# eBay/Sequence-Semantic-Embedding

Hardware: AMD Instinct MI355X
Metric: encoded seqs/sec (+ query x target cosine-scores/sec, top-1 vs ref) (higher is better)
Workload: dtype f32; 1 GPU; configs[1]: classification stand-in, dual-encoder LSTM H=S=256 E=50 T=32 V=32000; encode 16384 source seqs/GPU/step + cosine top-10 vs 571-target index; batch_per_gpu=16384, seq_len=32, targets=571, parallelism=dp1, weights=random-init (reference initialisers, seed 0)

## Files before the change

### sequence-semantic-embedding_amd/csrc/lstm_fwd.hip

```cpp
#include <cstdlib>
#include <type_traits>

#include "sse_kernels.h"

#define LSTM_THREADS 512
#define LSTM_BM 64

#ifdef SSE_FWD_CLOCK
#include <cstdio>
__device__ long long g_fwd_clk[16 * 8];
#define FW_CLK_DECL long long ck_[8] = {0, 0, 0, 0, 0, 0, 0, 0}, ck_t = clock64();
#define FW_CLK(i)                   \
  {                                 \
    const long long n_ = clock64(); \
    ck_[i] += n_ - ck_t;            \
    ck_t = n_;                      \
  }
#else
#define FW_CLK_DECL
#define FW_CLK(i)
#endif

bool lstm_fwd_x_double(int KGx, int KGh, int RT) { return (size_t)(2 * RT * (KGx + KGh) + 1) * 1024 <= 160 * 1024; }
size_t lstm_fwd_lds_bytes(int KGx, int KGh, int RT) {
  const int xb = lstm_fwd_x_double(KGx, KGh, RT) ? 2 : 1;
  return (size_t)(xb * RT * KGx + 2 * RT * KGh) * 256 * sizeof(float) + 64 * 4 * sizeof(float);
}
static size_t lstm_fwd_xt_lds_bytes(int KGh, int RT) { return (size_t)(2 * RT * KGh) * 256 * sizeof(float) + 64 * 4 * sizeof(float); }


typedef unsigned int u32x4 __attribute__((ext_vector_type(4)));

__device__ __forceinline__ f32x4 wload(__amdgpu_buffer_rsrc_t r, int voff, int soff) {
  return __builtin_bit_cast(f32x4, __builtin_amdgcn_raw_buffer_load_b128(r, voff, soff, 0));
}

struct NoTail {
  __device__ void operator()() const {}
};
template <int MT, bool LIN, bool SWAP, int R = (MT == 1 ? 4 : 3), bool PRIO = true, typename Tail = NoTail>
__device__ __forceinline__ void gemm_pass(__amdgpu_buffer_rsrc_t wr, int voff, int soff, const float *const (&xa)[MT],
                                          const float *const (&ha)[MT], int KGx, int kend, f32x16 (&acc)[MT][2], int kbeg = 0,
                                          const Tail &tail = Tail{}) {
  auto a_frag = [&](int m, int kg) -> f32x4 {
    if constexpr (LIN) return *reinterpret_cast<const f32x4 *>(xa[m] + kg * 256);
    return *reinterpret_cast<const f32x4 *>(kg < KGx ? xa[m] + kg * 256 : ha[m] + (kg - KGx) * 256);
  };
  f32x4 p0[R], p1[R], af[R][MT];
  const int klast = kend - 1;
#pragma unroll
  for (int s = 0; s < R; ++s) {
    const int kg = kbeg + s < kend ? kbeg + s : klast;
    p0[s] = wload(wr, voff, soff + kg * 4096);
// ... 7 lines not shown
    for (int e = 0; e < 4; ++e)
#pragma unroll
      for (int m = 0; m < MT; ++m) {
        acc[m][0] = SWAP ? __builtin_amdgcn_mfma_f32_32x32x2f32(p0[s][e], af[s][m][e], acc[m][0], 0, 0, 0)
                         : __builtin_amdgcn_mfma_f32_32x32x2f32(af[s][m][e], p0[s][e], acc[m][0], 0, 0, 0);
        acc[m][1] = SWAP ? __builtin_amdgcn_mfma_f32_32x32x2f32(p1[s][e], af[s][m][e], acc[m][1], 0, 0, 0)
                         : __builtin_amdgcn_mfma_f32_32x32x2f32(af[s][m][e], p1[s][e], acc[m][1], 0, 0, 0);
      }
  };
  if constexpr (PRIO) __builtin_amdgcn_s_setprio(1);
  int kg = kbeg;
  for (; kg + R <= kend; kg += R) {
#pragma unroll
    for (int s = 0; s < R; ++s) {
      __builtin_amdgcn_sched_barrier(0);
      mfmas(s);
      __builtin_amdgcn_sched_barrier(0);
      const int kn = (kg + s + R < kend) ? kg + s + R : klast;
      p0[s] = wload(wr, voff, soff + kn * 4096);
      p1[s] = wload(wr, voff + 1024, soff + kn * 4096);
#pragma unroll
      for (int m = 0; m < MT; ++m) af[s][m] = a_frag(m, kn);
    }
  }
  if constexpr (!std::is_same_v<Tail, NoTail>) {
    __builtin_amdgcn_sched_barrier(0);
    tail();
    __builtin_amdgcn_sched_barrier(0);
  }
#pragma unroll
  for (int s = 0; s < R - 1; ++s)
    if (kg + s < kend) mfmas(s);
  if constexpr (PRIO) __builtin_amdgcn_s_setprio(0);
}

template <int RT, int MT, int UBW, bool TRAIN, bool LIN, bool SPL = false, bool TSW = false, bool XT = false>
__global__ __launch_bounds__(LSTM_THREADS) void lstm_fwd_kernel(LstmFwdArgs a) {
  static_assert(!TSW || TRAIN, "TSW is the training forward in the inference orientation");
  static_assert(!XT || (!TRAIN && LIN && !SPL), "the x table is an inference path of the linear LDS layout");
  constexpr int NTHR = LSTM_THREADS;
  extern __shared__ __attribute__((aligned(16))) float smem[];
  constexpr int ROWS = RT * 32;
  constexpr int TPR = NTHR / ROWS;
  constexpr int NWR = 8 / RT;
  constexpr bool SWAP = !TRAIN || TSW;
  const int tid = threadIdx.x, lane = tid & 63, w = tid >> 6;
  const bool split3 = !TRAIN && RT == 2 && MT == 1 && a.H > 64 && a.H <= 96;
  int ub0 = (RT == 2 && MT == 1) ? (w >> 1) : w;
  int mt0 = (RT == 2 && MT == 1) ? (w & 1) : 0;
  bool do_a = true, do_b = true;
  if (split3 && w >= 4) {
    ub0 = 2;
    mt0 = (w - 4) >> 1;
    do_a = ((w & 1) == 0);
    do_b = !do_a;
  }
  if constexpr (SPL) {
    static_assert(RT == 1 && MT == 1 && UBW == 1, "pass-split mapping is defined for one 32-row tile");
    ub0 = w & 3;
    do_a = w < 4;
    do_b = !do_a;
  }
  const int fidx = SPL ? ub0 : mt0;
  const int KGx = a.KGx, KGh = a.KGh, KG = KGx + KGh, T = a.T;
  const int KGhe = (a.KGhe > 0 && a.KGhe < KGh) ? a.KGhe : KGh;
  const int KGxs = XT ? 0 : KGx, KGs = KGxs + KGh;
  constexpr bool XD = LIN;
  auto xptr = [&](int buf, int mt) -> float * {
    return LIN ? smem + (size_t)((buf * RT + mt) * KGs) * 256 : smem + (size_t)(mt * KGx) * 256;
  };
  auto hptr = [&](int buf, int mt) -> float * {
    return LIN ? smem + (size_t)((buf * RT + mt) * KGs + KGxs) * 256
               : smem + (size_t)(RT * KGx + (buf * RT + mt) * KGh) * 256;
  };
  float *red = smem + (size_t)(LIN ? 2 * RT * KGs : RT * KGx + 2 * RT * KGh) * 256;
  const int b0 = blockIdx.x * ROWS;
  int *pass_flag = reinterpret_cast<int *>(red + 16);
  if (tid < 8) pass_flag[tid] = 0;

// ... 13 lines not shown
  for (int m = 0; m < MT; ++m) {
    const int r = b0 + (mt0 + m) * 32 + (lane & 31);
    xt_row[m] = XT && r < a.B ? (a.row_map ? a.row_map[r] : r) : -1;
  }
  auto xt_id = [&](int m, int t) -> int { return xt_row[m] >= 0 ? a.ids[(size_t)xt_row[m] * T + t] : 0; };
  auto xt_check = [&](int id) -> int {
    if (id < 0 || id >= a.V) {
      atomicOr(a.err, 1);
      id = 0;
    }
    return id;
  };
  auto x_store = [&](int buf, int kg, f32x4 lo, f32x4 hi) {
    float *dst = xptr(buf, xr >> 5) + (size_t)kg * 256;
    *reinterpret_cast<f32x4 *>(dst + (xr & 31) * 4) = lo;
    *reinterpret_cast<f32x4 *>(dst + (32 + (xr & 31)) * 4) = hi;
  };

  const int NT32 = a.NT32 > 0 ? a.NT32 : gridDim.x * RT;
  auto tape_x = [&](int ts, int kg, f32x4 lo, f32x4 hi) {
    if constexpr (TSW) {
      if (kg >= 8) return;
      sse_quad_transpose(lo, lane);
      sse_quad_transpose(hi, lane);
      const int KT = 2 + KGh / 4, b = xr & 31;
      const size_t rg = ((size_t)ts * NT32 + blockIdx.x * RT + (xr >> 5)) * 4 + (b >> 3);
      const int k0 = kg * 8 + (xr & 3);
      float *dst = a.tape_a + (rg * KT + (k0 >> 5)) * 256 + ((((b >> 2) & 1) * 32 + (k0 & 31)) << 2);
      __builtin_nontemporal_store(lo, reinterpret_cast<f32x4 *>(dst));
      __builtin_nontemporal_store(hi, reinterpret_cast<f32x4 *>(dst + 16));
    }
  };

  int t0 = 0;
  if (!TRAIN && a.pad_h != nullptr) {
    int lead = T;
    if (row_ok) {
      for (int t = xq; t < T; t += TPR)
        if (id_row[t] != 0) {
          lead = t;
          break;
        }
    }
#pragma unroll
    for (int o = 32; o > 0; o >>= 1) lead = min(lead, __shfl_xor(lead, o));
    if (lane == 0) red[w] = __int_as_float(lead);
    __syncthreads();
    lead = T;
    for (int i = 0; i < NTHR / 64; ++i) lead = min(lead, __float_as_int(red[i]));
    t0 = min(lead, T - 1);
    __syncthreads();
  }

  int xid[MT];
#pragma unroll
  for (int m = 0; m < MT; ++m) xid[m] = XT ? xt_check(xt_id(m, t0)) : 0;
  if constexpr (!XT) {
    const int id = fetch_id(t0);
    const float *src = a.emb + (size_t)id * a.Ep;
    for (int kg = xq; kg < KGx; kg += TPR) {
      f32x4 lo = *reinterpret_cast<const f32x4 *>(src + kg * 8);
      f32x4 hi = *reinterpret_cast<const f32x4 *>(src + kg * 8 + 4);
      x_store(t0 & 1, kg, lo, hi);
    }
    if constexpr (TSW) {
      for (int kg = xq; kg < 8; kg += TPR) {
        f32x4 lo = {0, 0, 0, 0}, hi = {0, 0, 0, 0};
        if (kg < KGx) {
          lo = *reinterpret_cast<const f32x4 *>(src + kg * 8);
          hi = *reinterpret_cast<const f32x4 *>(src + kg * 8 + 4);
        }
        tape_x(t0, kg, lo, hi);
      }
    }
  }
  {
    const int Hp = KGh * 8;
    for (int i = tid; i < RT * KGh * 256; i += NTHR) {
      const int mt = i / (KGh * 256), e = i % (KGh * 256);
      const int un = (e >> 8) * 8 + ((e >> 7) & 1) * 4 + (e & 3);
      hptr(t0 & 1, mt)[e] = (t0 > 0) ? a.pad_h[(size_t)t0 * Hp + un] : 0.0f;
    }
  }

  f32x16 c[UBW][MT];
#pragma unroll
  for (int u = 0; u < UBW; ++u) {
#pragma unroll
    for (int r = 0; r < 16; ++r) {
      const int un = (ub0 + 8 * u) * 32 + (SWAP ? mfma_row(r, lane) : (lane & 31));
      const float c0 = (t0 > 0) ? a.pad_c[(size_t)t0 * (KGh * 8) + un] : 0.0f;
#pragma unroll
      for (int m = 0; m < MT; ++m) c[u][m][r] = c0;
    }
  }

  if constexpr (TSW) {
    if (do_b) {
      const int KT = 2 + KGh / 4, b = lane & 31;
#pragma unroll
      for (int u = 0; u < UBW; ++u)
#pragma unroll
        for (int m = 0; m < MT; ++m) {
          const size_t rg = ((size_t)t0 * NT32 + blockIdx.x * RT + mt0 + m) * 4 + (b >> 3);
#pragma unroll
          for (int q4 = 0; q4 < 4; ++q4) {
            float *dst = a.tape_a + (rg * KT + 2 + ub0 + 8 * u) * 256 + ((((b >> 2) & 1) * 32 + q4 * 8 + (lane >> 5) * 4 + (b & 3)) << 2);
            __builtin_nontemporal_store(f32x4{0, 0, 0, 0}, reinterpret_cast<f32x4 *>(dst));
          }
        }
    }
  }
  __syncthreads();

  const __amdgpu_buffer_rsrc_t wr = __builtin_amdgcn_make_buffer_rsrc(
      const_cast<float *>(a.Wp), 0, (KGh / 4) * KG * 4096, 0x00020000);
  const int wvoff = lane * 16;
  const __amdgpu_buffer_rsrc_t xtr = __builtin_amdgcn_make_buffer_rsrc(
      const_cast<float *>(a.xtab), 0, XT ? a.V * a.xtab_ub * 512 : 0, 0x00020000);
  auto xt_load = [&](f32x16(&acc)[MT][2], const int (&id)[MT], int ub, int q) {
    const int soff = __builtin_amdgcn_readfirstlane(ub * 512 + q * 128);
#pragma unroll
    for (int m = 0; m < MT; ++m) {
      const int voff = id[m] * (a.xtab_ub * 512) + (lane >> 5) * 64;
#pragma unroll
      for (int i = 0; i < 4; ++i) {
        const f32x4 v0 = wload(xtr, voff + 16 * i, soff), v1 = wload(xtr, voff + 128 + 16 * i, soff);
#pragma unroll
        for (int e = 0; e < 4; ++e) {
          acc[m][0][4 * i + e] = v0[e];
          acc[m][1][4 * i + e] = v1[e];
        }
      }
    }
  };

  auto acc_init = [&](f32x16(&acc)[MT][2], const int (&id)[MT], int ub, int q) {
    if constexpr (XT) {
      xt_load(acc, id, ub, q);
    } else {
#pragma unroll
      for (int m = 0; m < MT; ++m)
#pragma unroll
        for (int r = 0; r < 16; ++r) {
          acc[m][0][r] = 0.0f;
          acc[m][1][r] = 0.0f;
        }
    }
  };

  constexpr bool PF = XT && RT == 2 && MT == 2 && UBW == 1;
  const bool live0 = !(a.H > 0 && ub0 * 32 >= a.H);
  f32x16 ga[MT][2], gb[MT][2];
  if (PF && live0) xt_load(ga, xid, ub0, 0);

  FW_CLK_DECL
  for (int t = t0; t < T; ++t) {
    FW_CLK(0)
    const bool have_next = (t + 1) < T;
    int nid = 0;
    f32x4 nlo = {0, 0, 0, 0}, nhi = {0, 0, 0, 0};
    int xnid[MT];
#pragma unroll
    for (int m = 0; m < MT; ++m) xnid[m] = XT && have_next ? xt_id(m, t + 1) : 0;
    if (!XT && have_next) {
      nid = fetch_id(t + 1);
      if (xq < KGx) {
        const float *src = a.emb + (size_t)nid * a.Ep + xq * 8;
        nlo = *reinterpret_cast<const f32x4 *>(src);
        nhi = *reinterpret_cast<const f32x4 *>(src + 4);
      }
    }

    const int cur = t & 1, nxt = (t + 1) & 1;
    const float *xa[MT], *ha[MT];
#pragma unroll
    for (int m = 0; m < MT; ++m) {
      xa[m] = xptr(cur, mt0 + m) + lane * 4;
      ha[m] = hptr(cur, mt0 + m) + lane * 4;
    }

    if constexpr (TRAIN && !TSW) {
      const int KT = 2 + KGh / 4;
      const int nk = 64 + KGh * 8;
      auto a_elem = [&](int mt, int kp, int b) -> float {
        if (kp >= 64) {
          const int un = kp - 64;
          return hptr(cur, mt)[(size_t)(un >> 3) * 256 + ((((un >> 2) & 1) * 32 + b) << 2) + (un & 3)];
// ... 207 lines not shown
              cn4[e] = cn;
            }
            if constexpr (TRAIN) {
              __builtin_nontemporal_store(sf4, reinterpret_cast<f32x4 *>(tp[m] + 2048 + q4 * 256));
              __builtin_nontemporal_store(so4, reinterpret_cast<f32x4 *>(tp[m] + 3072 + q4 * 256));
              __builtin_nontemporal_store(cn4, reinterpret_cast<f32x4 *>(tp[m] + 4096 + q4 * 256));
            }
          }
        }
      }
    }

    FW_CLK(6)
    if (XD) {
      __syncthreads();
      FW_CLK(7)
#pragma unroll
      for (int m = 0; m < MT; ++m)
        if (XT && !(PF && live0) && have_next) xid[m] = xt_check(xnid[m]);
    } else {
      __syncthreads();
      if (have_next) {
        if (xq < KGx) x_store(0, xq, nlo, nhi);
        for (int kg = xq + TPR; kg < KGx; kg += TPR) {
          const float *src = a.emb + (size_t)nid * a.Ep + kg * 8;
          x_store(0, kg, *reinterpret_cast<const f32x4 *>(src), *reinterpret_cast<const f32x4 *>(src + 4));
        }
        tape_x(t + 1, xq, nlo, nhi);
      }
      __syncthreads();
    }
  }

#ifdef SSE_FWD_CLOCK
  if (blockIdx.x == 0 && lane == 0)
    for (int i = 0; i < 8; ++i) g_fwd_clk[w * 8 + i] = ck_[i];
#endif
  if constexpr (TRAIN) {
    const int Hp = KGh * 8;
    for (int i = tid; i < ROWS * Hp; i += NTHR) {
      const int un = i % Hp, b = i / Hp;
      a.h_last[(size_t)(b0 + b) * Hp + un] =
          hptr(T & 1, b >> 5)[(size_t)(un >> 3) * 256 + ((((un >> 2) & 1) * 32 + (b & 31)) << 2) + (un & 3)];
    }
  }

  const int wn = w % NWR, wm = w / NWR;
  constexpr bool pwave = true;
  constexpr int PT = 16 / NWR;
  const float *hp = hptr(T & 1, wm) + lane * 4;
  f32x16 pacc[PT];
  float *ssq = hptr((T + 1) & 1, 0);
#pragma unroll
  for (int i = 0; i < PT; ++i) {
    const int nt = wn + NWR * i;
#pragma unroll
    for (int r = 0; r < 16; ++r) pacc[i][r] = 0.0f;
    if (nt < a.NTS && pwave) {
      const float *mp = a.Mp + (size_t)nt * KGh * 256 + lane * 4;
      f32x4 ax = *reinterpret_cast<const f32x4 *>(hp), bx = *reinterpret_cast<const f32x4 *>(mp), ay, by;
      int kg = 0;
      for (; kg + 1 < KGhe; kg += 2) {
        ay = *reinterpret_cast<const f32x4 *>(hp + (kg + 1) * 256);
        by = *reinterpret_cast<const f32x4 *>(mp + (kg + 1) * 256);
        __builtin_amdgcn_sched_barrier(0);
#pragma unroll
        for (int e = 0; e < 4; ++e) pacc[i] = __builtin_amdgcn_mfma_f32_32x32x2f32(ax[e], bx[e], pacc[i], 0, 0, 0);
        __builtin_amdgcn_sched_barrier(0);
        const int k2 = (kg + 2 < KGhe) ? kg + 2 : kg;
        ax = *reinterpret_cast<const f32x4 *>(hp + k2 * 256);
        bx = *reinterpret_cast<const f32x4 *>(mp + k2 * 256);
        __builtin_amdgcn_sched_barrier(0);
#pragma unroll
        for (int e = 0; e < 4; ++e) pacc[i] = __builtin_amdgcn_mfma_f32_32x32x2f32(ay[e], by[e], pacc[i], 0, 0, 0);
        __builtin_amdgcn_sched_barrier(0);
      }
      if (kg < KGhe) {
#pragma unroll
        for (int e = 0; e < 4; ++e) pacc[i] = __builtin_amdgcn_mfma_f32_32x32x2f32(ax[e], bx[e], pacc[i], 0, 0, 0);
      }
      if (a.normalize) {
#pragma unroll
        for (int r = 0; r < 16; ++r) {
          float v = pacc[i][r] * pacc[i][r];
          v += __shfl_xor(v, 1);
          v += __shfl_xor(v, 2);
          v += __shfl_xor(v, 4);
          v += __shfl_xor(v, 8);
          v += __shfl_xor(v, 16);
          if ((lane & 31) == 0) ssq[(wm * 32 + mfma_row(r, lane)) * 16 + nt] = v;
        }
      }
    }
  }
  float scale[16];
  if (a.normalize) {
    __syncthreads();
#pragma unroll
    for (int r = 0; r < 16; ++r) {
      const float *pr = ssq + (wm * 32 + mfma_row(r, lane)) * 16;
      float tot = 0.0f;
      for (int j = 0; j < a.NTS; ++j) tot += pr[j];
      scale[r] = 1.0f / sqrtf(fmaxf(tot, 1e-12f));
    }
  } else {
#pragma unroll
    for (int r = 0; r < 16; ++r) scale[r] = 1.0f;
  }
#pragma unroll
  for (int i = 0; i < PT; ++i) {
    const int nt = wn + NWR * i;
    const int col = nt * 32 + (lane & 31);
    if (nt < a.NTS && col < a.S && pwave) {
#pragma unroll
      for (int r = 0; r < 16; ++r) {
        const int row = b0 + wm * 32 + mfma_row(r, lane);
        if (row < a.B) a.out[(size_t)(a.row_map ? a.row_map[row] : row) * a.S + col] = pacc[i][r] * scale[r];
      }
    }
  }
}

template <int RT, int MT, int UBW, bool TRAIN, bool LIN, bool SPL, bool TSW = false, bool XT = false>
static hipError_t launch_one(const LstmFwdArgs &a, size_t lds, hipStream_t stream) {
  hipError_t e = hipFuncSetAttribute(reinterpret_cast<const void *>(lstm_fwd_kernel<RT, MT, UBW, TRAIN, LIN, SPL, TSW, XT>),
                                     hipFuncAttributeMaxDynamicSharedMemorySize, (int)lds);
  if (e != hipSuccess) return e;
  const dim3 grid(a.NT32 > 0 ? a.NT32 / RT : (a.B + RT * 32 - 1) / (RT * 32)), block(LSTM_THREADS);
  hipLaunchKernelGGL((lstm_fwd_kernel<RT, MT, UBW, TRAIN, LIN, SPL, TSW, XT>), grid, block, lds, stream, a);
#ifdef SSE_FWD_CLOCK
  {
    static int n = 0;
    if (a.B >= 1024 && n++ % 16 == 4) {
      long long v[128];
      (void)hipStreamSynchronize(stream);
      (void)hipMemcpyFromSymbol(v, HIP_SYMBOL(g_fwd_clk), sizeof v);
      for (int w = 0; w < 8; ++w)
        fprintf(stderr, "[fwd clock <%d,%d,%d> B=%d H=%d] wave %d cycles/step: prefetch %lld | setup %lld | passA gemm %lld | epiA+x %lld | passB gemm %lld | flag wait %lld | epiB %lld | barrier %lld\n",
                RT, MT, UBW, a.B, a.H, w, v[w * 8 + 0] / a.T, v[w * 8 + 1] / a.T, v[w * 8 + 2] / a.T, v[w * 8 + 3] / a.T, v[w * 8 + 4] / a.T, v[w * 8 + 5] / a.T,
                v[w * 8 + 6] / a.T, v[w * 8 + 7] / a.T);
    }
  }
#endif
  return hipGetLastError();
}

template <int RT, int MT, int UBW, bool SPL = false>
static hipError_t launch_cfg(const LstmFwdArgs &a_in, hipStream_t stream) {
  LstmFwdArgs a = a_in;
  a.xdouble = lstm_fwd_x_double(a.KGx, a.KGh, RT) ? 1 : 0;
  const size_t lds = lstm_fwd_lds_bytes(a.KGx, a.KGh, RT);
  const bool train = a.tape_g != nullptr;
  if constexpr (!SPL && !(RT == 2 && MT == 1)) {
    if (!train && a.xtab != nullptr) {
      if (a.xtab_ub != (a.H > 0 ? (a.H + 31) / 32 : a.KGh / 4)) return hipErrorInvalidValue;
      if ((int64_t)a.V * a.xtab_ub * 512 > INT32_MAX) return hipErrorInvalidValue;
      return launch_one<RT, MT, UBW, false, true, false, false, true>(a, lstm_fwd_xt_lds_bytes(a.KGh, RT), stream);
    }
  }
  if (train && a.tape_swap) {
    if (a.tape_a_split) return hipErrorInvalidValue;
    return a.xdouble ? launch_one<RT, MT, UBW, true, true, SPL, true>(a, lds, stream)
                     : launch_one<RT, MT, UBW, true, false, SPL, true>(a, lds, stream);
  }
  if (a.xdouble)
    return train ? launch_one<RT, MT, UBW, true, true, SPL>(a, lds, stream) : launch_one<RT, MT, UBW, false, true, SPL>(a, lds, stream);
  return train ? launch_one<RT, MT, UBW, true, false, SPL>(a, lds, stream) : launch_one<RT, MT, UBW, false, false, SPL>(a, lds, stream);
}

int lstm_fwd_rows_per_wg(int Hp, int B, int tiles_elsewhere, int cus) {
  if (cus <= 0) cus = 256;
  if (Hp == 512) return 32;
  if ((Hp == 256 || Hp == 128) && (B + 31) / 32 + tiles_elsewhere <= cus) return 32;
// ... 40 lines not shown
```

### sequence-semantic-embedding_amd/csrc/sse_api.hip

```cpp
#include <cmath>
#include <cstdarg>
#include <cstdio>
#include <cstdlib>
#include <algorithm>
#include <chrono>
#include <cstring>
#include <dlfcn.h>
#include <link.h>
#include <mutex>
#include <string>
#include <vector>

#include "../../include/sse_hip.h"
#include "sse_kernels.h"
#include "train.h"

namespace {

thread_local std::string g_create_error;

struct Variable {
  std::string name;
  int rows = 0, cols = 0;
  int64_t count = 0;
// ... 65 lines not shown
  DevBuf ids_raw[2], perm, hot_part[2];
  int perm_B = 0;
  std::vector<int32_t> h_perm, h_rows[2], h_tgt;
  std::vector<float> h_labels;
};

}

enum { PATH_PERSIST, PATH_CLUSTER, PATH_SMALL, PATH_X3, PATH_GENERIC, PATH_FWD, PATH_FWD_ROWS32, PATH_FWD_ROWS64, PATH_FWD_GS, PATH_FWD_XT,
       PATH_COUNT };
static const char *const LSTM_PATH_NAMES[PATH_COUNT] = {"lstm_path_persist", "lstm_path_cluster", "lstm_path_small", "lstm_path_x3",
                                                "lstm_path_generic", "lstm_path_fwd", "lstm_fwd_rows32", "lstm_fwd_rows64",
                                                "lstm_fwd_gate_split", "lstm_fwd_x_table"};

struct sse_handle {
  sse_config cfg;
  std::mutex mu;
  std::string err;
  std::vector<Variable> vars;
  Encoder enc[2];
  bool packed_dirty = true;
  uint64_t weights_version = 1;
  bool mp_fresh = false;
  bool pad_skip = true;
  int pad_sort_dev = 1;
  int64_t score_two_pass_min_rows = 49152, score_two_pass_rows = 524288;
  int64_t two_pass_calls = 0;
  DevBuf s_lmax;
  bool lstm_gate_split = true;
  DevBuf s_padzero, s_padwork, s_padorder;
  int32_t *pad_stat = nullptr;
  int32_t pad_seq = 0;
  int64_t pad_sorted_calls = 0;
  int64_t lstm_path_calls[10] = {0, 0, 0, 0, 0, 0, 0, 0, 0, 0};
  bool lstm_x3 = false;
  unsigned short *emb16 = nullptr;
  bool emb16_valid = false;
  int lstm_persist_rows = 32;
  uint32_t persist_epoch = 0;
  hipStream_t stream = nullptr;
  bool persist_inject = false;
  int64_t persist_fallbacks = 0;
  int cu_count = 0;
  int lstm_cluster_rows = 1024;
  uint32_t cluster_epoch = 0;
  int lstm_cluster_chunks = 3;
  int cluster_backoff = -1;
  int cluster_skip[2] = {0, 0};
  int lstm_cluster_coop = 1;
  int lstm_cluster_wt = 0;
  int lstm_cluster_drop = 0;
  int lstm_small_rows = 1024;
  int lstm_x_table = 1;
  int lstm_x_table_mb = 256;
  int64_t x_table_builds = 0;
  bool score_small_index = true;
  bool score_small_x3 = true;
  bool score_bf16 = true;
  void *idxp16 = nullptr;
  size_t idxp16_cap = 0;
  bool idxp16_valid = false;
  bool fb_cnt_init = false;
  int uncert_word = 0;
  bool cnn_bf16 = false;
  unsigned short *emb_bf16 = nullptr, *cnn_Wc16 = nullptr, *cnn_Mx3 = nullptr;
  int lstm_train_rows = 0;
// ... 391 lines not shown

static int encode_generic_locked(sse_handle *h, Encoder &e, const int32_t *ids, int B, int T, int normalize, float *out, hipStream_t st) {
  const sse_config &c = h->cfg;
  const int E = c.embedding_size, S = c.encoding_size;
  const GenLstmDims d0 = gen_lstm_dims(32, T, E, e.H);
  const size_t per_row = (size_t)T * d0.Kp * sizeof(float);
  int rows = (int)std::min<size_t>(8192, std::max<size_t>(32, (((size_t)1 << 30) / per_row) / 32 * 32));
  const GenLstmDims dm = gen_lstm_dims(std::min(rows, B), T, E, e.H);
  if (reserve(h, h->g_A, gen_lstm_a_floats(dm) * sizeof(float)) || reserve(h, h->g_G, (size_t)dm.Bp * 4 * dm.Hq * sizeof(float)) ||
      reserve(h, h->g_c, (size_t)dm.Bp * dm.Hq * sizeof(float)) || reserve(h, h->g_hl, (size_t)dm.Bp * dm.Hq * sizeof(float)) ||
      reserve(h, h->g_raw, (size_t)dm.Bp * S * sizeof(float)))
    return 1;
  const int side = (&e == &h->enc[1]) ? 1 : 0;
  if (h->g_ver[side] != h->weights_version || !h->g_KT[side].p) {
    if (reserve(h, h->g_KT[side], gen_lstm_kt_floats(dm) * sizeof(float)) || reserve(h, h->g_Kq[side], gen_lstm_kt_floats(dm) * sizeof(float)) ||
        reserve(h, h->g_MT[side], (size_t)S * dm.Hq * sizeof(float)))
      return 1;
    HIPCHECK(h, launch_gen_pack(h->vars[e.kernel].dev, h->vars[e.proj].dev, dm, S, (float *)h->g_KT[side].p, (float *)h->g_Kq[side].p,
                                (float *)h->g_MT[side].p, st));
    h->g_ver[side] = h->weights_version;
  }
  for (int b0 = 0; b0 < B; b0 += rows) {
    const int nb = std::min(rows, B - b0);
    const GenLstmDims d = gen_lstm_dims(nb, T, E, e.H);
    HIPCHECK(h, launch_gen_forward(ids + (size_t)b0 * T, h->vars[0].dev, c.vocab_size, (const float *)h->g_KT[side].p, h->vars[e.bias].dev, d,
                                   (float *)h->g_A.p, (float *)h->g_G.p, (float *)h->g_c.p, nullptr, (float *)h->g_hl.p, h->err_flag, st));
    HIPCHECK(h, launch_gen_project((const float *)h->g_hl.p, (const float *)h->g_MT[side].p, d, S, (float *)h->g_raw.p, st));
    if (normalize) HIPCHECK(h, launch_l2_normalize((const float *)h->g_raw.p, out + (size_t)b0 * S, nb, S, st));
    else HIPCHECK(h, hipMemcpyAsync(out + (size_t)b0 * S, h->g_raw.p, (size_t)nb * S * sizeof(float), hipMemcpyDeviceToDevice, st));
  }
  return 0;
}

static int device_pad_sort(sse_handle *h, int side, const int32_t *ids, int B, int T, hipStream_t st, const int32_t **row_map,
                           bool *padded) {
  if (*row_map || !h->pad_skip || h->pad_sort_dev == 0 || T < 2 || T > SSE_PAD_SORT_MAX_T || B <= 64) return 0;
  volatile int32_t *stat = h->pad_stat + 2 * side;
  const int seen = h->pad_sort_dev == 2 ? 2 : (stat[0] != 0 ? (int)stat[1] : 1);
  const bool scatter = seen != 0;
  if (!h->s_padzero.p) {
    if (reserve(h, h->s_padzero, pad_sort_zeroed_words() * sizeof(int32_t))) return 1;
    HIPCHECK(h, hipMemsetAsync(h->s_padzero.p, 0, h->s_padzero.cap, st));
  }
  if (reserve(h, h->s_padwork, pad_sort_work_words(B, T) * sizeof(int32_t))) return 1;
  if (scatter && reserve(h, h->s_padorder, (size_t)B * sizeof(int32_t))) return 1;
  h->pad_seq = h->pad_seq == INT32_MAX ? 1 : h->pad_seq + 1;
  HIPCHECK(h, launch_pad_sort(ids, B, T, (int32_t *)h->s_padzero.p, (int32_t *)h->s_padwork.p, (int32_t *)h->s_padorder.p,
                              h->pad_stat + 2 * side, h->pad_seq, scatter, st));
  if (scatter) {
    *row_map = (const int32_t *)h->s_padorder.p;
    *padded = seen == 2;
    h->pad_sorted_calls += 1;
  }
  return 0;
}

int next_epoch(sse_handle *h, DevBuf &xchg, uint32_t &epoch, size_t need, hipStream_t st, uint32_t *next) {
  if (epoch == 0 || epoch >= (1u << 20) - 1 || need > xchg.cap) {
    if (reserve(h, xchg, need)) return 1;
    HIPCHECK(h, hipMemsetAsync(xchg.p, 0, xchg.cap, st));
    epoch = 0;
  }
  *next = ++epoch;
  return 0;
}

int inject_miss(sse_handle *h, hipStream_t st) {
  static const int32_t four = 4;
  if (h->persist_inject) HIPCHECK(h, hipMemcpyAsync(h->err_flag, &four, sizeof four, hipMemcpyHostToDevice, st));
  return 0;
}

int encode_persist(sse_handle *h, int side, const int32_t *ids, int B, int T, int normalize, float *out, hipStream_t st) {
  Encoder &e = h->enc[side], &own = lstm_owner(h, e);
  if (ensure_waug(h, own, st)) return 1;
  LstmPersistArgs pa;
  fill_small_args(h, e, pa);
  pa.ids = ids;
  pa.out = out;
// ... 139 lines not shown
  if (h->lstm_x_table == 0 || own.Hp < 256) return 0;
  const int64_t V = h->cfg.vocab_size;
  const int UBt = (own.H + 31) / 32;
  const size_t bytes = lstm_xtable_floats(V, UBt) * sizeof(float);
  if (bytes > ((size_t)h->lstm_x_table_mb << 20) || bytes > (size_t)INT32_MAX) return 0;
  if (own.xtab_valid) {
    *use = true;
    return 0;
  }
  if (h->lstm_x_table == 1 && (int64_t)B * T < V) return 0;
  if (!own.xtab && hipMalloc((void **)&own.xtab, bytes) != hipSuccess) {
    (void)hipGetLastError();
    own.xtab = nullptr;
    return 0;
  }
  HIPCHECK(h, launch_lstm_xtable(h->emb_pad, own.Wp, V, own.Ep, own.KGx, own.KGh, UBt, own.xtab, st));
  own.xtab_valid = true;
  h->x_table_builds += 1;
  *use = true;
  return 0;
}

int encode_fwd(sse_handle *h, int side, const int32_t *ids, int B, int T, int normalize, float *out, const EncodeRequest &rq,
               hipStream_t st) {
  Encoder &e = h->enc[side], &own = lstm_owner(h, e);
  LstmFwdArgs a;
  fill_fwd_args(h, e, a);
  a.ids = ids;
  a.out = out;
  a.B = B;
  a.T = T;
  a.normalize = normalize ? 1 : 0;
  a.row_map = rq.row_map;
  bool padded_hint = rq.padded_hint;
  if (device_pad_sort(h, side, ids, B, T, st, &a.row_map, &padded_hint)) return 1;
  if (h->pad_skip && T > 1) {
    if (ensure_pad_table(h, own.pad_fwd, own.Hp, T, st, [&](const int32_t *zero_ids, float *scratch, int Tt) {
          LstmFwdArgs ta;
          fill_fwd_args(h, own, ta);
          ta.ids = zero_ids;
          ta.out = scratch;
          ta.B = 1;
          ta.T = Tt;
          ta.normalize = 0;
          ta.rec_h = own.pad_fwd.h;
          ta.rec_c = own.pad_fwd.c;
          HIPCHECK(h, launch_lstm_fwd(ta, own.Hp, st));
          return 0;
        }))
      return 1;
    a.pad_h = own.pad_fwd.h;
    a.pad_c = own.pad_fwd.c;
    if (padded_hint && a.row_map && e.Hp <= 256) a.force_rows = 32;
  }
  bool use_xt = false;
  if (ensure_x_table(h, own, B, T, st, &use_xt)) return 1;
  if (use_xt) {
    a.xtab = own.xtab;
    a.xtab_ub = (own.H + 31) / 32;
  }
  const int variant = lstm_fwd_variant(a, e.Hp);
  h->lstm_path_calls[(variant & 64) ? PATH_FWD_ROWS64 : PATH_FWD_ROWS32] += 1;
  if (variant & LSTM_FWD_GATE_SPLIT) h->lstm_path_calls[PATH_FWD_GS] += 1;
  if (variant & LSTM_FWD_X_TABLE) h->lstm_path_calls[PATH_FWD_XT] += 1;
  HIPCHECK(h, launch_lstm_fwd(a, e.Hp, st));
  return 0;
}

int encode_dev_locked(sse_handle *h, int side, const int32_t *ids, int B, int T, int normalize, float *out, hipStream_t st,
                      const EncodeRequest &rq = EncodeRequest()) {
  const sse_config &c = h->cfg;
  if (side != SSE_SIDE_SOURCE && side != SSE_SIDE_TARGET) return fail(h, "side must be 0 (source) or 1 (target)");
  if (B < 0 || T < 1) return fail(h, "bad batch shape B=%d T=%d", B, T);
  if (B == 0) return 0;
  if (side == SSE_SIDE_TARGET && h->tgt_table >= 0) {
    const Variable &tv = h->vars[h->tgt_table];
    if (B != tv.rows)
      return fail(h, "network mode has no target sequence encoder: tgt_seq_embedding is a [%d,%d] variable "
                     "(sse_model.py:214,233); request exactly %d rows", tv.rows, tv.cols, tv.rows);
    if (normalize) HIPCHECK(h, launch_l2_normalize(tv.dev, out, tv.rows, tv.cols, st));
    else HIPCHECK(h, hipMemcpyAsync(out, tv.dev, tv.count * sizeof(float), hipMemcpyDeviceToDevice, st));
    return 0;
  }
  if (c.network_mode == SSE_MODE_SOURCE_ONLY_CNN) {
    if (ensure_packed(h, st)) return 1;
    const int Ep = emb_cols(c);
    if (T < 5) return fail(h, "source_only_cnn needs max_seq_length >= 5 (widest filter)");
    if (cnn_lds_bytes(T, Ep, 0) > 160 * 1024)
      return fail(h, "source_only_cnn: T*E = %d*%d does not fit the LDS tile of the gfx950 kernel", T, c.embedding_size);
    if (reserve(h, h->s_feat, (size_t)((B + 31) / 32) * 72 * 256 * sizeof(float))) return 1;
    if (h->cnn_bf16) {
      const int Ep8 = round_up(c.embedding_size, 8);
      if (cnn_bf16_lds_bytes(T, Ep8, 0) > 160 * 1024)
        return fail(h, "source_only_cnn (bf16): T*E = %d*%d does not fit the LDS tile of the gfx950 kernel", T, c.embedding_size);
      HIPCHECK(h, launch_cnn_fwd_bf16(ids, h->emb_bf16, h->cnn_Wc16, h->cnn_bias, (float *)h->s_feat.p, h->err_flag, B, T,
                                      c.vocab_size, Ep8, nullptr, nullptr, st));
      HIPCHECK(h, launch_cnn_proj_x3((const float *)h->s_feat.p, h->cnn_Mx3, out, B, c.encoding_size, normalize ? 1 : 0, st));
// ... 1083 lines not shown
  if (B == 0) return 0;
  if (B < 0 || T < 1 || !ids_host || !out_scores || !out_ids) return fail(h, "bad arguments to sse_encode_score_topk");
  if (!h->idxp) return fail(h, "no index uploaded");
  if (h->cfg.encoding_size != h->idx_S)
    return fail(h, "index dimension %d != encoding_size %d", h->idx_S, h->cfg.encoding_size);
  if (encode_host_ids_locked(h, side, ids_host, B, T, normalize, true)) return 1;
  int32_t bits = 0;
  if (score_to_host_locked(h, (const float *)h->s_out.p, B, k, out_scores, out_ids, &bits)) return 1;
  if (bits) {
    if (check_err_flag(h, nullptr, &bits)) return 1;
    if (bits == 4) {
      if (encode_fallback_locked(h, side, B, T, normalize, nullptr)) return 1;
      if (score_to_host_locked(h, (const float *)h->s_out.p, B, k, out_scores, out_ids)) return 1;
    }
  }
  if (enc_out_host)
    HIPCHECK(h, hipMemcpy(enc_out_host, h->s_out.p, (size_t)B * h->cfg.encoding_size * sizeof(float), hipMemcpyDeviceToHost));
  return 0;
}

int sse_get_counter(sse_handle *h, const char *name, int64_t *value) {
  if (!h || !name || !value) return 1;
  std::lock_guard<std::mutex> lk(h->mu);
  if (strcmp(name, "lstm_persist_fallbacks") == 0) {
    *value = h->persist_fallbacks;
    return 0;
  }
  if (strcmp(name, "score_two_pass_calls") == 0) {
    *value = h->two_pass_calls;
    return 0;
  }
  if (strcmp(name, "pad_sorted_calls") == 0) {
    *value = h->pad_sorted_calls;
    return 0;
  }
  if (strcmp(name, "eval_paired_calls") == 0) {
    *value = h->eval_paired_calls;
    return 0;
  }
  if (strcmp(name, "lstm_x_table_builds") == 0) {
    *value = h->x_table_builds;
    return 0;
  }
  for (int i = 0; i < PATH_COUNT; ++i) {
    if (strcmp(name, LSTM_PATH_NAMES[i]) != 0) continue;
    *value = h->lstm_path_calls[i];
    return 0;
  }
  if (strcmp(name, "lstm_coop_refused") == 0) {
    *value = (int64_t)lstm_coop_refused();
    return 0;
  }
  static const char *const rank_names[2] = {"score_rank_band_rows", "score_rank_bruteforce_pairs"};
  for (int i = 0; i < 2; ++i) {
    if (strcmp(name, rank_names[i]) != 0) continue;
    unsigned long long v[2] = {0, 0};
    if (h->s_rk_cnt.p && h->rk_cnt_init) {
      HIPCHECK(h, hipSetDevice(h->cfg.device));
      HIPCHECK(h, hipDeviceSynchronize());
      HIPCHECK(h, hipMemcpy(v, h->s_rk_cnt.p, sizeof v, hipMemcpyDeviceToHost));
    }
    *value = (int64_t)v[i];
    return 0;
  }
  static const char *const above_names[3] = {"score_above_band_rows", "score_above_bruteforce_pairs", "score_above_long_segments"};
  for (int i = 0; i < 3; ++i) {
// ... 1485 lines not shown
```

### sequence-semantic-embedding_amd/csrc/sse_kernels.h

```cpp
#pragma once
#include <hip/hip_runtime.h>
#include <stdint.h>

typedef float f32x4 __attribute__((ext_vector_type(4)));
typedef float f32x16 __attribute__((ext_vector_type(16)));

__host__ __device__ static inline int frag32_off(int r_in_tile, int k_in_group) {
  return ((((k_in_group >> 2) << 5) + r_in_tile) << 2) + (k_in_group & 3);
}

__device__ static inline int mfma_row(int reg, int lane) { return (reg & 3) + 8 * (reg >> 2) + 4 * (lane >> 5); }

static inline int round_up(int x, int m) { return (x + m - 1) / m * m; }

typedef unsigned int sse_u32x4 __attribute__((ext_vector_type(4)));
__host__ __device__ static inline unsigned short sse_bf16_rne(float f) {
  unsigned u;
  __builtin_memcpy(&u, &f, 4);
  u += 0x7FFFu + ((u >> 16) & 1u);
  return (unsigned short)(u >> 16);
}
__host__ __device__ static inline float sse_bf16_f32(unsigned short h) {
  const unsigned u = (unsigned)h << 16;
  float f;
// ... 47 lines not shown
  (void)v;
  (void)lane;
#endif
}

#define SSE_TANH_SMALL 0.25f
__device__ __forceinline__ float sse_sigmoid(float x) { return __builtin_amdgcn_rcpf(1.0f + __builtin_amdgcn_exp2f(-1.44269504089f * x)); }
__device__ __forceinline__ float sse_tanh(float x) {
  const float big = 1.0f - 2.0f * __builtin_amdgcn_rcpf(1.0f + __builtin_amdgcn_exp2f(2.88539008178f * x));
  const float x2 = x * x;
  const float p = __builtin_fmaf(x2, __builtin_fmaf(x2, __builtin_fmaf(x2, -17.0f / 315.0f, 2.0f / 15.0f), -1.0f / 3.0f), 1.0f);
  return __builtin_fabsf(x) < SSE_TANH_SMALL ? x * p : big;
}

struct LstmFwdArgs {
  const int32_t *ids;
  const float *emb;
  const float *Wp;
  const float *Mp;
  float *out;
  int32_t *err;
  int32_t B, T, V, Ep, KGx, KGh, S, NTS, normalize;
  int32_t H = 0;
  int32_t KGhe = 0;
  int32_t NT32 = 0;
  int32_t xdouble = 1;
  int32_t tiles_elsewhere = 0;
  int32_t force_rows = 0;
  int32_t cu_count = 0;
  int32_t gate_split = 1;
  const float *pad_h = nullptr, *pad_c = nullptr;
  const int32_t *row_map = nullptr;
  float *rec_h = nullptr, *rec_c = nullptr;
  const float *xtab = nullptr;
  int32_t xtab_ub = 0;
  float *tape_g = nullptr;
  float *tape_a = nullptr;
  int32_t tape_a_split = 0;
  int32_t tape_swap = 0;
  float *h_last = nullptr;
};
size_t lstm_fwd_lds_bytes(int KGx, int KGh, int RT);
bool lstm_fwd_x_double(int KGx, int KGh, int RT);
int lstm_fwd_rows_per_wg(int Hp, int B, int tiles_elsewhere = 0, int cus = 0 );
hipError_t launch_lstm_fwd(const LstmFwdArgs &a, int Hp, hipStream_t stream);
enum { LSTM_FWD_GATE_SPLIT = 1, LSTM_FWD_X_TABLE = 2 };
int lstm_fwd_variant(const LstmFwdArgs &a, int Hp);
size_t lstm_xtable_floats(int64_t V, int UBt);
hipError_t launch_lstm_xtable(const float *emb , const float *Wp, int64_t V, int Ep, int KGx, int KGh, int UBt,
                              float *table, hipStream_t stream);
size_t lstm_fwd_gs_lds_bytes(int KGx, int NB);
bool lstm_fwd_gs_ok(int KGx, int KGh, int H);
hipError_t launch_lstm_fwd_gs(const LstmFwdArgs &a, hipStream_t stream);

struct LstmSmallArgs {
  const int32_t *ids;
  const float *emb;
  const float *Waug;
  const float *M;
  float *out;
  int32_t *err;
  int32_t B, T, V, E, H, S, normalize;
  const float *pad_h = nullptr, *pad_c = nullptr;
  float *rec_h = nullptr, *rec_c = nullptr;
  int32_t pad_stride = 0;
};
size_t lstm_small_lds_bytes(int E, int H, int S);
size_t lstm_small_waug_floats(int E, int H);
hipError_t launch_pack_lstm_small(const float *K, const float *b, int E, int H, float *out, hipStream_t stream);
hipError_t launch_lstm_small(const LstmSmallArgs &a, hipStream_t stream);

struct LstmX3Args {
  const int32_t *ids;
  const unsigned short *emb16;
  const unsigned short *Wx3;
  const float *Mp;
  float *out;
  int32_t *err;
  int32_t B, T, V, KGX, H, S, NTS, normalize;
  const int32_t *row_map = nullptr;
// ... 324 lines not shown
```

Baseline: 7.573 million seqs/s.

## Fold pad detection into LSTM forward and pipeline the output projection

When the pad-sort pass would only detect padding without scattering, detection now happens inside the LSTM forward kernel, which writes the pad status flag itself. This removes a separate detection kernel launch. The prologue also hoists the id loads and the x-table setup ahead of the pad scan, unrolls that scan four ids at a time, and zeroes the h state with vector stores when no prefix is skipped. The final projection moves to a multi-stage buffer-load pipeline with DPP row reductions. The trade-offs are added kernel complexity, a system fence on the flag write, and extra clock instrumentation behind a debug macro.

```diff
diff --git a/sequence-semantic-embedding_amd/csrc/lstm_fwd.hip b/sequence-semantic-embedding_amd/csrc/lstm_fwd.hip
--- a/sequence-semantic-embedding_amd/csrc/lstm_fwd.hip
+++ b/sequence-semantic-embedding_amd/csrc/lstm_fwd.hip
@@ -16,9 +16,21 @@
     ck_[i] += n_ - ck_t;            \
     ck_t = n_;                      \
   }
+__device__ long long g_fwd_fix[16 * 8];
+#define FX_CLK_DECL long long fx_[8] = {0, 0, 0, 0, 0, 0, 0, 0}, fx_t = clock64();
+#define FX_CLK(i)                   \
+  {                                 \
+    const long long n_ = clock64(); \
+    fx_[i] += n_ - fx_t;            \
+    fx_t = n_;                      \
+  }
+#define FX_DRAIN asm volatile("s_waitcnt vmcnt(0)" ::: "memory");
 #else
 #define FW_CLK_DECL
 #define FW_CLK(i)
+#define FX_CLK_DECL
+#define FX_CLK(i)
+#define FX_DRAIN
 #endif
 
 bool lstm_fwd_x_double(int KGx, int KGh, int RT) { return (size_t)(2 * RT * (KGx + KGh) + 1) * 1024 <= 160 * 1024; }
@@ -92,6 +104,54 @@
   for (int s = 0; s < R - 1; ++s)
     if (kg + s < kend) mfmas(s);
   if constexpr (PRIO) __builtin_amdgcn_s_setprio(0);
+}
+
+__device__ __forceinline__ float row_sum16_lane0(float v) {
+  auto dpp = [](float x, auto ctrl) {
+    return __builtin_bit_cast(float, __builtin_amdgcn_update_dpp(0, __builtin_bit_cast(int, x), decltype(ctrl)::value, 0xf, 0xf, true));
+  };
+  v += dpp(v, std::integral_constant<int, 0xB1>{});
+  v += dpp(v, std::integral_constant<int, 0x4E>{});
+  v += dpp(v, std::integral_constant<int, 0x104>{});
+  v += dpp(v, std::integral_constant<int, 0x108>{});
+  return v;
+}
+
+template <int NL, int PT, int R = (NL <= 2 ? 4 : 3)>
+__device__ __forceinline__ void proj_pass(__amdgpu_buffer_rsrc_t mr, int voff, int soff, int sstride, const float *hp, int kend,
+                                          f32x16 (&pacc)[PT]) {
+  static_assert(NL >= 1 && NL <= PT, "live N tiles of a wave");
+  f32x4 hf[R], mf[R][NL];
+  const int klast = kend - 1;
+  auto load = [&](int s, int kg) {
+    hf[s] = *reinterpret_cast<const f32x4 *>(hp + kg * 256);
+#pragma unroll
+    for (int i = 0; i < NL; ++i) mf[s][i] = wload(mr, voff, soff + i * sstride + kg * 1024);
+  };
+#pragma unroll
+  for (int s = 0; s < R; ++s) {
+    load(s, s < kend ? s : klast);
+    __builtin_amdgcn_sched_barrier(0);
+  }
+  auto mfmas = [&](int s) {
+#pragma unroll
+    for (int e = 0; e < 4; ++e)
+#pragma unroll
+      for (int i = 0; i < NL; ++i) pacc[i] = __builtin_amdgcn_mfma_f32_32x32x2f32(hf[s][e], mf[s][i][e], pacc[i], 0, 0, 0);
+  };
+  int kg = 0;
+  for (; kg + R <= kend; kg += R) {
+#pragma unroll
+    for (int s = 0; s < R; ++s) {
+      __builtin_amdgcn_sched_barrier(0);
+      mfmas(s);
+      __builtin_amdgcn_sched_barrier(0);
+      load(s, (kg + s + R < kend) ? kg + s + R : klast);
+    }
+  }
+#pragma unroll
+  for (int s = 0; s < R - 1; ++s)
+    if (kg + s < kend) mfmas(s);
 }
 
 template <int RT, int MT, int UBW, bool TRAIN, bool LIN, bool SPL = false, bool TSW = false, bool XT = false>
@@ -105,6 +165,7 @@
   constexpr int NWR = 8 / RT;
   constexpr bool SWAP = !TRAIN || TSW;
   const int tid = threadIdx.x, lane = tid & 63, w = tid >> 6;
+  FX_CLK_DECL
   const bool split3 = !TRAIN && RT == 2 && MT == 1 && a.H > 64 && a.H <= 96;
   int ub0 = (RT == 2 && MT == 1) ? (w >> 1) : w;
   int mt0 = (RT == 2 && MT == 1) ? (w & 1) : 0;
@@ -184,15 +245,68 @@
     }
   };
 
+  const __amdgpu_buffer_rsrc_t wr = __builtin_amdgcn_make_buffer_rsrc(
+      const_cast<float *>(a.Wp), 0, (KGh / 4) * KG * 4096, 0x00020000);
+  const int wvoff = lane * 16;
+  const __amdgpu_buffer_rsrc_t xtr = __builtin_amdgcn_make_buffer_rsrc(
+      const_cast<float *>(a.xtab), 0, XT ? a.V * a.xtab_ub * 512 : 0, 0x00020000);
+  auto xt_load = [&](f32x16(&acc)[MT][2], const int (&id)[MT], int ub, int q) {
+    const int soff = __builtin_amdgcn_readfirstlane(ub * 512 + q * 128);
+#pragma unroll
+    for (int m = 0; m < MT; ++m) {
+      const int voff = id[m] * (a.xtab_ub * 512) + (lane >> 5) * 64;
+#pragma unroll
+      for (int i = 0; i < 4; ++i) {
+        const f32x4 v0 = wload(xtr, voff + 16 * i, soff), v1 = wload(xtr, voff + 128 + 16 * i, soff);
+#pragma unroll
+        for (int e = 0; e < 4; ++e) {
+          acc[m][0][4 * i + e] = v0[e];
+          acc[m][1][4 * i + e] = v1[e];
+        }
+      }
+    }
+  };
+
+  constexpr bool PF = XT && RT == 2 && MT == 2 && UBW == 1;
+  const bool live0 = !(a.H > 0 && ub0 * 32 >= a.H);
+  f32x16 ga[MT][2], gb[MT][2];
+  int xid[MT];
+  const bool scan = !TRAIN && a.pad_h != nullptr;
+#pragma unroll
+  for (int m = 0; m < MT; ++m) xid[m] = XT ? xt_id(m, 0) : 0;
+  const int id_first = (!XT && row_ok) ? id_row[0] : 0;
+  int sv[4] = {1, 1, 1, 1};
+  if constexpr (!TRAIN) {
+#pragma unroll
+    for (int j = 0; j < 4; ++j) sv[j] = id_row[min(xq + j * TPR, T - 1)];
+  }
+  __builtin_amdgcn_sched_barrier(0);
+#pragma unroll
+  for (int m = 0; m < MT; ++m) xid[m] = XT ? xt_check(xid[m]) : 0;
+  __builtin_amdgcn_sched_barrier(0);
+
   int t0 = 0;
-  if (!TRAIN && a.pad_h != nullptr) {
+  if (scan) {
     int lead = T;
+    bool first_pad = false;
     if (row_ok) {
-      for (int t = xq; t < T; t += TPR)
-        if (id_row[t] != 0) {
-          lead = t;
-          break;
-        }
+      first_pad = xq == 0 && sv[0] == 0;
+#pragma unroll
+      for (int j = 3; j >= 0; --j)
+        if (xq + j * TPR < T && sv[j] != 0) lead = xq + j * TPR;
+      for (int tb = xq + 4 * TPR; tb < T && lead == T; tb += 4 * TPR) {
+        int v[4];
+#pragma unroll
+        for (int j = 0; j < 4; ++j) v[j] = id_row[min(tb + j * TPR, T - 1)];
+#pragma unroll
+        for (int j = 3; j >= 0; --j)
+          if (tb + j * TPR < T && v[j] != 0) lead = tb + j * TPR;
+      }
+    }
+    if (a.det_stat != nullptr && __ballot(first_pad) != 0 && lane == 0) {
+      a.det_stat[1] = 1;
+      __threadfence_system();
+      a.det_stat[0] = a.det_seq;
     }
 #pragma unroll
     for (int o = 32; o > 0; o >>= 1) lead = min(lead, __shfl_xor(lead, o));
@@ -203,12 +317,18 @@
     t0 = min(lead, T - 1);
     __syncthreads();
   }
-
-  int xid[MT];
-#pragma unroll
-  for (int m = 0; m < MT; ++m) xid[m] = XT ? xt_check(xt_id(m, t0)) : 0;
+  FX_CLK(0)
+
+  if (XT && t0 > 0) {
+#pragma unroll
+    for (int m = 0; m < MT; ++m) xid[m] = xt_check(xt_id(m, t0));
+  }
   if constexpr (!XT) {
-    const int id = fetch_id(t0);
+    int id = t0 > 0 ? (row_ok ? id_row[t0] : 0) : id_first;
+    if (id < 0 || id >= a.V) {
+      atomicOr(a.err, 1);
+      id = 0;
+    }
     const float *src = a.emb + (size_t)id * a.Ep;
     for (int kg = xq; kg < KGx; kg += TPR) {
       f32x4 lo = *reinterpret_cast<const f32x4 *>(src + kg * 8);
@@ -226,7 +346,13 @@
       }
     }
   }
-  {
+  if (t0 == 0) {
+#pragma unroll
+    for (int mt = 0; mt < RT; ++mt) {
+      float *hz = hptr(0, mt);
+      for (int i = tid * 4; i < KGh * 256; i += NTHR * 4) *reinterpret_cast<f32x4 *>(hz + i) = f32x4{0, 0, 0, 0};
+    }
+  } else {
     const int Hp = KGh * 8;
     for (int i = tid; i < RT * KGh * 256; i += NTHR) {
       const int mt = i / (KGh * 256), e = i % (KGh * 256);
@@ -264,28 +390,7 @@
     }
   }
   __syncthreads();
-
-  const __amdgpu_buffer_rsrc_t wr = __builtin_amdgcn_make_buffer_rsrc(
-      const_cast<float *>(a.Wp), 0, (KGh / 4) * KG * 4096, 0x00020000);
-  const int wvoff = lane * 16;
-  const __amdgpu_buffer_rsrc_t xtr = __builtin_amdgcn_make_buffer_rsrc(
-      const_cast<float *>(a.xtab), 0, XT ? a.V * a.xtab_ub * 512 : 0, 0x00020000);
-  auto xt_load = [&](f32x16(&acc)[MT][2], const int (&id)[MT], int ub, int q) {
-    const int soff = __builtin_amdgcn_readfirstlane(ub * 512 + q * 128);
-#pragma unroll
-    for (int m = 0; m < MT; ++m) {
-      const int voff = id[m] * (a.xtab_ub * 512) + (lane >> 5) * 64;
-#pragma unroll
-      for (int i = 0; i < 4; ++i) {
-        const f32x4 v0 = wload(xtr, voff + 16 * i, soff), v1 = wload(xtr, voff + 128 + 16 * i, soff);
-#pragma unroll
-        for (int e = 0; e < 4; ++e) {
-          acc[m][0][4 * i + e] = v0[e];
-          acc[m][1][4 * i + e] = v1[e];
-        }
-      }
-    }
-  };
+  FX_CLK(1)
 
   auto acc_init = [&](f32x16(&acc)[MT][2], const int (&id)[MT], int ub, int q) {
     if constexpr (XT) {
@@ -301,11 +406,9 @@
     }
   };
 
-  constexpr bool PF = XT && RT == 2 && MT == 2 && UBW == 1;
-  const bool live0 = !(a.H > 0 && ub0 * 32 >= a.H);
-  f32x16 ga[MT][2], gb[MT][2];
   if (PF && live0) xt_load(ga, xid, ub0, 0);
-
+  FX_DRAIN
+  FX_CLK(2)
   FW_CLK_DECL
   for (int t = t0; t < T; ++t) {
     FW_CLK(0)
@@ -579,6 +682,7 @@
     }
   }
 
+  FX_CLK(3)
 #ifdef SSE_FWD_CLOCK
   if (blockIdx.x == 0 && lane == 0)
     for (int i = 0; i < 8; ++i) g_fwd_clk[w * 8 + i] = ck_[i];
@@ -593,53 +697,41 @@
   }
 
   const int wn = w % NWR, wm = w / NWR;
-  constexpr bool pwave = true;
   constexpr int PT = 16 / NWR;
   const float *hp = hptr(T & 1, wm) + lane * 4;
   f32x16 pacc[PT];
   float *ssq = hptr((T + 1) & 1, 0);
 #pragma unroll
-  for (int i = 0; i < PT; ++i) {
-    const int nt = wn + NWR * i;
+  for (int i = 0; i < PT; ++i)
 #pragma unroll
     for (int r = 0; r < 16; ++r) pacc[i][r] = 0.0f;
-    if (nt < a.NTS && pwave) {
-      const float *mp = a.Mp + (size_t)nt * KGh * 256 + lane * 4;
-      f32x4 ax = *reinterpret_cast<const f32x4 *>(hp), bx = *reinterpret_cast<const f32x4 *>(mp), ay, by;
-      int kg = 0;
-      for (; kg + 1 < KGhe; kg += 2) {
-        ay = *reinterpret_cast<const f32x4 *>(hp + (kg + 1) * 256);
-        by = *reinterpret_cast<const f32x4 *>(mp + (kg + 1) * 256);
-        __builtin_amdgcn_sched_barrier(0);
-#pragma unroll
-        for (int e = 0; e < 4; ++e) pacc[i] = __builtin_amdgcn_mfma_f32_32x32x2f32(ax[e], bx[e], pacc[i], 0, 0, 0);
-        __builtin_amdgcn_sched_barrier(0);
-        const int k2 = (kg + 2 < KGhe) ? kg + 2 : kg;
-        ax = *reinterpret_cast<const f32x4 *>(hp + k2 * 256);
-        bx = *reinterpret_cast<const f32x4 *>(mp + k2 * 256);
-        __builtin_amdgcn_sched_barrier(0);
-#pragma unroll
-        for (int e = 0; e < 4; ++e) pacc[i] = __builtin_amdgcn_mfma_f32_32x32x2f32(ay[e], by[e], pacc[i], 0, 0, 0);
-        __builtin_amdgcn_sched_barrier(0);
-      }
-      if (kg < KGhe) {
-#pragma unroll
-        for (int e = 0; e < 4; ++e) pacc[i] = __builtin_amdgcn_mfma_f32_32x32x2f32(ax[e], bx[e], pacc[i], 0, 0, 0);
-      }
-      if (a.normalize) {
+  const int nl = __builtin_amdgcn_readfirstlane(a.NTS > wn ? min((a.NTS - wn + NWR - 1) / NWR, PT) : 0);
+  {
+    const __amdgpu_buffer_rsrc_t mr = __builtin_amdgcn_make_buffer_rsrc(const_cast<float *>(a.Mp), 0, a.NTS * KGh * 1024, 0x00020000);
+    const int msoff = __builtin_amdgcn_readfirstlane(wn) * KGh * 1024, mstride = NWR * KGh * 1024;
+    if (nl == 1) proj_pass<1, PT>(mr, lane * 16, msoff, mstride, hp, KGhe, pacc);
+    else if (nl == 2) proj_pass<2, PT>(mr, lane * 16, msoff, mstride, hp, KGhe, pacc);
+    if constexpr (PT == 4) {
+      if (nl == 3) proj_pass<3, PT>(mr, lane * 16, msoff, mstride, hp, KGhe, pacc);
+      else if (nl == 4) proj_pass<4, PT>(mr, lane * 16, msoff, mstride, hp, KGhe, pacc);
+    }
+  }
+  if (a.normalize) {
+#pragma unroll
+    for (int i = 0; i < PT; ++i) {
+      const int nt = wn + NWR * i;
+      if (i < nl) {
 #pragma unroll
         for (int r = 0; r < 16; ++r) {
           float v = pacc[i][r] * pacc[i][r];
-          v += __shfl_xor(v, 1);
-          v += __shfl_xor(v, 2);
-          v += __shfl_xor(v, 4);
-          v += __shfl_xor(v, 8);
+          v = row_sum16_lane0(v);
           v += __shfl_xor(v, 16);
           if ((lane & 31) == 0) ssq[(wm * 32 + mfma_row(r, lane)) * 16 + nt] = v;
         }
       }
     }
   }
+  FX_CLK(4)
   float scale[16];
   if (a.normalize) {
     __syncthreads();
@@ -654,11 +746,12 @@
 #pragma unroll
     for (int r = 0; r < 16; ++r) scale[r] = 1.0f;
   }
+  FX_CLK(5)
 #pragma unroll
   for (int i = 0; i < PT; ++i) {
     const int nt = wn + NWR * i;
     const int col = nt * 32 + (lane & 31);
-    if (nt < a.NTS && col < a.S && pwave) {
+    if (nt < a.NTS && col < a.S) {
 #pragma unroll
       for (int r = 0; r < 16; ++r) {
         const int row = b0 + wm * 32 + mfma_row(r, lane);
@@ -666,6 +759,12 @@
       }
     }
   }
+  FX_DRAIN
+  FX_CLK(6)
+#ifdef SSE_FWD_CLOCK
+  if (blockIdx.x == 0 && lane == 0)
+    for (int i = 0; i < 8; ++i) g_fwd_fix[w * 8 + i] = fx_[i];
+#endif
 }
 
 template <int RT, int MT, int UBW, bool TRAIN, bool LIN, bool SPL, bool TSW = false, bool XT = false>
@@ -686,6 +785,10 @@
         fprintf(stderr, "[fwd clock <%d,%d,%d> B=%d H=%d] wave %d cycles/step: prefetch %lld | setup %lld | passA gemm %lld | epiA+x %lld | passB gemm %lld | flag wait %lld | epiB %lld | barrier %lld\n",
                 RT, MT, UBW, a.B, a.H, w, v[w * 8 + 0] / a.T, v[w * 8 + 1] / a.T, v[w * 8 + 2] / a.T, v[w * 8 + 3] / a.T, v[w * 8 + 4] / a.T, v[w * 8 + 5] / a.T,
                 v[w * 8 + 6] / a.T, v[w * 8 + 7] / a.T);
+      (void)hipMemcpyFromSymbol(v, HIP_SYMBOL(g_fwd_fix), sizeof v);
+      for (int w = 0; w < 8; ++w)
+        fprintf(stderr, "[fwd fixed <%d,%d,%d> B=%d H=%d T=%d] wave %d cycles: pad scan %lld | prologue barrier %lld | table fragment, loop entry %lld | loop %lld | projection %lld | normalise %lld | stores %lld\n",
+                RT, MT, UBW, a.B, a.H, a.T, w, v[w * 8 + 0], v[w * 8 + 1], v[w * 8 + 2], v[w * 8 + 3], v[w * 8 + 4], v[w * 8 + 5], v[w * 8 + 6]);
     }
   }
 #endif
diff --git a/sequence-semantic-embedding_amd/csrc/sse_api.hip b/sequence-semantic-embedding_amd/csrc/sse_api.hip
--- a/sequence-semantic-embedding_amd/csrc/sse_api.hip
+++ b/sequence-semantic-embedding_amd/csrc/sse_api.hip
@@ -121,6 +121,7 @@
   int32_t *pad_stat = nullptr;
   int32_t pad_seq = 0;
   int64_t pad_sorted_calls = 0;
+  int64_t pad_detect_launches = 0;
   int64_t lstm_path_calls[10] = {0, 0, 0, 0, 0, 0, 0, 0, 0, 0};
   bool lstm_x3 = false;
   unsigned short *emb16 = nullptr;
@@ -578,8 +579,14 @@
   return 0;
 }
 
+static int launch_pad_detect(sse_handle *h, int side, const int32_t *ids, int B, int T, hipStream_t st) {
+  HIPCHECK(h, launch_pad_sort(ids, B, T, (int32_t *)h->s_padzero.p, (int32_t *)h->s_padwork.p, (int32_t *)h->s_padorder.p,
+                              h->pad_stat + 2 * side, h->pad_seq, false, st));
+  h->pad_detect_launches += 1;
+  return 0;
+}
 static int device_pad_sort(sse_handle *h, int side, const int32_t *ids, int B, int T, hipStream_t st, const int32_t **row_map,
-                           bool *padded) {
+                           bool *padded, bool *fold = nullptr) {
   if (*row_map || !h->pad_skip || h->pad_sort_dev == 0 || T < 2 || T > SSE_PAD_SORT_MAX_T || B <= 64) return 0;
   volatile int32_t *stat = h->pad_stat + 2 * side;
   const int seen = h->pad_sort_dev == 2 ? 2 : (stat[0] != 0 ? (int)stat[1] : 1);
@@ -591,6 +598,11 @@
   if (reserve(h, h->s_padwork, pad_sort_work_words(B, T) * sizeof(int32_t))) return 1;
   if (scatter && reserve(h, h->s_padorder, (size_t)B * sizeof(int32_t))) return 1;
   h->pad_seq = h->pad_seq == INT32_MAX ? 1 : h->pad_seq + 1;
+  if (!scatter) {
+    if (fold) *fold = true;
+    else if (launch_pad_detect(h, side, ids, B, T, st)) return 1;
+    return 0;
+  }
   HIPCHECK(h, launch_pad_sort(ids, B, T, (int32_t *)h->s_padzero.p, (int32_t *)h->s_padwork.p, (int32_t *)h->s_padorder.p,
                               h->pad_stat + 2 * side, h->pad_seq, scatter, st));
   if (scatter) {
@@ -796,8 +808,8 @@
   a.T = T;
   a.normalize = normalize ? 1 : 0;
   a.row_map = rq.row_map;
-  bool padded_hint = rq.padded_hint;
-  if (device_pad_sort(h, side, ids, B, T, st, &a.row_map, &padded_hint)) return 1;
+  bool padded_hint = rq.padded_hint, fold_detect = false;
+  if (device_pad_sort(h, side, ids, B, T, st, &a.row_map, &padded_hint, &fold_detect)) return 1;
   if (h->pad_skip && T > 1) {
     if (ensure_pad_table(h, own.pad_fwd, own.Hp, T, st, [&](const int32_t *zero_ids, float *scratch, int Tt) {
           LstmFwdArgs ta;
@@ -827,6 +839,14 @@
   h->lstm_path_calls[(variant & 64) ? PATH_FWD_ROWS64 : PATH_FWD_ROWS32] += 1;
   if (variant & LSTM_FWD_GATE_SPLIT) h->lstm_path_calls[PATH_FWD_GS] += 1;
   if (variant & LSTM_FWD_X_TABLE) h->lstm_path_calls[PATH_FWD_XT] += 1;
+  if (fold_detect) {
+    if (lstm_fwd_detects(a, variant)) {
+      a.det_stat = h->pad_stat + 2 * side;
+      a.det_seq = h->pad_seq;
+    } else if (launch_pad_detect(h, side, ids, B, T, st)) {
+      return 1;
+    }
+  }
   HIPCHECK(h, launch_lstm_fwd(a, e.Hp, st));
   return 0;
 }
@@ -1976,6 +1996,10 @@
   }
   if (strcmp(name, "pad_sorted_calls") == 0) {
     *value = h->pad_sorted_calls;
+    return 0;
+  }
+  if (strcmp(name, "pad_detect_launches") == 0) {
+    *value = h->pad_detect_launches;
     return 0;
   }
   if (strcmp(name, "eval_paired_calls") == 0) {
diff --git a/sequence-semantic-embedding_amd/csrc/sse_kernels.h b/sequence-semantic-embedding_amd/csrc/sse_kernels.h
--- a/sequence-semantic-embedding_amd/csrc/sse_kernels.h
+++ b/sequence-semantic-embedding_amd/csrc/sse_kernels.h
@@ -103,6 +103,8 @@
   const float *pad_h = nullptr, *pad_c = nullptr;
   const int32_t *row_map = nullptr;
   float *rec_h = nullptr, *rec_c = nullptr;
+  volatile int32_t *det_stat = nullptr;
+  int32_t det_seq = 0;
   const float *xtab = nullptr;
   int32_t xtab_ub = 0;
   float *tape_g = nullptr;
@@ -117,6 +119,9 @@
 hipError_t launch_lstm_fwd(const LstmFwdArgs &a, int Hp, hipStream_t stream);
 enum { LSTM_FWD_GATE_SPLIT = 1, LSTM_FWD_X_TABLE = 2 };
 int lstm_fwd_variant(const LstmFwdArgs &a, int Hp);
+inline bool lstm_fwd_detects(const LstmFwdArgs &a, int variant) {
+  return !(variant & LSTM_FWD_GATE_SPLIT) && a.tape_g == nullptr && a.pad_h != nullptr;
+}
 size_t lstm_xtable_floats(int64_t V, int UBt);
 hipError_t launch_lstm_xtable(const float *emb , const float *Wp, int64_t V, int Ep, int KGx, int KGh, int UBt,
                               float *table, hipStream_t stream);
```

Result: no change. 7.616 million seqs/s (median of 6 runs) (+0.6%).
